# AntoineRichard/MoonSuperResolution

Hardware: AMD Instinct MI355X
Metric: 512x512 DEM tiles/s (whole job) (higher is better)
Workload: dtype f16 main term + fp8 / fp6 cross terms in the chip-filling convs, bf16x3 elsewhere (f32 in/out/accumulate; parity mode); 1 GPU; SPADE-512 GauGAN(512,8,256) batch=8 512x512 tiles per step (BASELINE configs[2]); image_size=512, batch_size=8, variant=gaugan, weights=random-init (Keras default distributions), seed 1234, parallelism=tile-sharded x1, streams_per_gpu=1

## Files before the change

### moonsuperresolution_amd/csrc/conv_sw.hip

```cpp
#include "conv_common.h"

namespace msr {

struct SwGeom {
    int tiles_x, tiles_y, tiles_n, tiles_mn;
    int walk_pb, walk_nb;
};

static constexpr int SW_HW = 18, SW_HP = 18 * 18, SW_BKP = 40, SW_HPB = SW_HP * SW_BKP;
#ifdef MSR_SW_STAMPS
static constexpr size_t SW_LDS = (size_t)3 * SW_HPB * sizeof(float) + 8192;
#else
static constexpr size_t SW_LDS = (size_t)3 * SW_HPB * sizeof(float);
#endif

template <int EPI, int OS>
__device__ __forceinline__ void sw_epilogue_body(const ConvParams& p, const SwGeom& g, f32x4 (&acc)[16][2], int wq, int lane,
                                                 int n0, int tx0, int ty0, int b0) {
    const int px = lane & 15, cg = lane >> 4;
    const int x = tx0 + px;
    const int cb0 = n0 + (wq >> 1) * 64 + (wq & 1) * 16 + 4 * cg;
    float* const obase = p.out + (size_t)p.out_off + (size_t)b0 * p.out_pb + x * p.out_px;
    if constexpr (EPI == EPI_SPADE) {
        const int ch = ((n0 + (wq >> 1) * 64) >> 1) + (wq & 1) * 16 + 4 * cg;
        const float4 gq4 = *reinterpret_cast<const float4*>(p.bias + cb0);
        const float4 bq4 = *reinterpret_cast<const float4*>(p.bias + cb0 + 32);
        const float4 mq4 = *reinterpret_cast<const float4*>(p.mean + ch);
        const float4 sq4 = *reinterpret_cast<const float4*>(p.stdv + ch);
        const float gq[4] = {gq4.x, gq4.y, gq4.z, gq4.w}, bq[4] = {bq4.x, bq4.y, bq4.z, bq4.w};
        const float mq[4] = {mq4.x, mq4.y, mq4.z, mq4.w};
        float sq[4] = {sq4.x, sq4.y, sq4.z, sq4.w};
        constexpr bool split = OS != OUT_F32;
        if constexpr (split) {
#pragma unroll
            for (int k = 0; k < 4; ++k) sq[k] = 1.f / sq[k];
        }
        const float* const abase = p.aux + (size_t)b0 * p.aux_pb + (x >> p.aux_shift) * p.aux_px + ch;
#pragma unroll
        for (int i0 = 0; i0 < 16; i0 += 8) {
            float4 xin[8];
#pragma unroll
            for (int ii = 0; ii < 8; ++ii)
                xin[ii] = *reinterpret_cast<const float4*>(abase + ((ty0 + i0 + ii) >> p.aux_shift) * p.aux_py);
#pragma unroll
            for (int ii = 0; ii < 8; ++ii) {
                const int i = i0 + ii;
                float* orow = obase + (ty0 + i) * p.out_py;
                const float xq[4] = {xin[ii].x, xin[ii].y, xin[ii].z, xin[ii].w};
                float v[4];
#pragma unroll
                for (int k = 0; k < 4; ++k) {
                    const float normalized = split ? (xq[k] - mq[k]) * sq[k] : (xq[k] - mq[k]) / sq[k];
                    const float t = (acc[i][0][k] + gq[k]) * normalized + (acc[i][1][k] + bq[k]);
                    v[k] = t >= 0.f ? t : t * p.slope;
                }
                if constexpr (OS == OUT_F16C) msr_store_f16c4_dev(orow, ch, v[0], v[1], v[2], v[3]);
                else if constexpr (OS == OUT_BF16X3) msr_store_split4_dev(orow, ch, v[0], v[1], v[2], v[3]);
                else *reinterpret_cast<float4*>(orow + ch) = make_float4(v[0], v[1], v[2], v[3]);
            }
        }
    } else {
#pragma unroll
        for (int j = 0; j < 2; ++j) {
            const int col = cb0 + 32 * j;
            const float4 b4 = *reinterpret_cast<const float4*>(p.bias + col);
            const float bq[4] = {b4.x, b4.y, b4.z, b4.w};
#pragma unroll
            for (int q4 = 0; q4 < 4; ++q4) {
                float4 res[4];
                if constexpr (EPI == EPI_RES) {
                    const float* abase = p.aux + (size_t)b0 * p.aux_pb + (x >> p.aux_shift) * p.aux_px + col;
#pragma unroll
                    for (int ii = 0; ii < 4; ++ii)
                        res[ii] = *reinterpret_cast<const float4*>(abase + ((ty0 + q4 * 4 + ii) >> p.aux_shift) * p.aux_py);
                }
                float s1[4] = {0.f, 0.f, 0.f, 0.f}, s2[4] = {0.f, 0.f, 0.f, 0.f}, pv[4];
#pragma unroll
                for (int ii = 0; ii < 4; ++ii) {
                    const int i = q4 * 4 + ii;
                    float d[4];
#pragma unroll
                    for (int k = 0; k < 4; ++k) d[k] = acc[i][j][k];
                    if constexpr (EPI == EPI_RES) { d[0] += res[ii].x; d[1] += res[ii].y; d[2] += res[ii].z; d[3] += res[ii].w; }
                    *reinterpret_cast<float4*>(obase + (ty0 + i) * p.out_py + col) =
                        make_float4(d[0] + bq[0], d[1] + bq[1], d[2] + bq[2], d[3] + bq[3]);
#pragma unroll
                    for (int k = 0; k < 4; ++k) {
                        if (ii == 0) pv[k] = d[k];
                        const float e = d[k] - pv[k];
                        s1[k] += e; s2[k] += e * e;
                    }
                }
                if (p.stat_partial) {
                    float mean[4], m2[4];
#pragma unroll
                    for (int k = 0; k < 4; ++k) {
                        const float mu = row16_sum(4.f * pv[k] + s1[k]) * (1.f / 64.f);
                        const float dl = (pv[k] - mu) + s1[k] * 0.25f;
                        const float t = row16_sum(s2[k] - s1[k] * s1[k] * 0.25f + 4.f * dl * dl);
                        mean[k] = bq[k] + mu;
                        m2[k] = t > 0.f ? t : 0.f;
                    }
                    if (px == 0) {
                        const int st = (b0 * (g.tiles_y * 2) + ((ty0 + q4 * 4) >> 3)) * g.tiles_x + (tx0 >> 4);
                        float* o = p.stat_partial + (size_t)(st * 2 + (q4 & 1)) * 3 * p.N + col;
                        *reinterpret_cast<float4*>(o) = make_float4(64.f, 64.f, 64.f, 64.f);
                        *reinterpret_cast<float4*>(o + p.N) = make_float4(mean[0], mean[1], mean[2], mean[3]);
                        *reinterpret_cast<float4*>(o + 2 * p.N) = make_float4(m2[0], m2[1], m2[2], m2[3]);
                    }
                }
            }
        }
    }
}

template <int EPI>
__device__ __forceinline__ void sw_epilogue(const ConvParams& p, const SwGeom& g, f32x4 (&acc)[16][2], int wq, int lane,
                                            int n0, int tx0, int ty0, int b0) {
    if constexpr (EPI == EPI_SPADE) {
        if (p.out_split == OUT_F16C) sw_epilogue_body<EPI, OUT_F16C>(p, g, acc, wq, lane, n0, tx0, ty0, b0);
        else if (p.out_split == OUT_BF16X3) sw_epilogue_body<EPI, OUT_BF16X3>(p, g, acc, wq, lane, n0, tx0, ty0, b0);
        else sw_epilogue_body<EPI, OUT_F32>(p, g, acc, wq, lane, n0, tx0, ty0, b0);
    } else {
        sw_epilogue_body<EPI, OUT_F32>(p, g, acc, wq, lane, n0, tx0, ty0, b0);
    }
}

#ifdef SW_NOBAR
#define SW_BARRIER() {}
#else
#define SW_BARRIER()                                           \
    {                                                          \
        __builtin_amdgcn_fence(__ATOMIC_RELEASE, "workgroup"); \
        __builtin_amdgcn_s_barrier();                          \
        __builtin_amdgcn_fence(__ATOMIC_ACQUIRE, "workgroup"); \
    }
#endif
#ifndef SW_UNROLL2
#define SW_UNROLL2 1
#endif
#ifndef SW_PD
#define SW_PD 6
#endif
#ifndef SW_PDC
#define SW_PDC 3
#endif

template <int EPI, bool F6 = false, bool NOX = false>
__global__ void __launch_bounds__(256) __attribute__((amdgpu_waves_per_eu(1, 1)))
conv_igemm_f16c_sw(const ConvParams p, const SwGeom g) {
    MSR_SATURATING_CONVERSIONS();
    constexpr int HW = SW_HW, HP = SW_HP, BKP = SW_BKP, HPB = SW_HPB;
    constexpr int NTHR = 256, BKC = 32;
    constexpr int H_ITEMS = (HP * 8 + NTHR - 1) / NTHR;
    static_assert(H_ITEMS == 11, "halo staging is written for 11 items per thread");
    constexpr int PD = SW_PD;
    constexpr int PDC = SW_PDC;
    constexpr int HD = 3;

    extern __shared__ __attribute__((aligned(16))) float smem[];

    const int tid = threadIdx.x;
    const int lane = tid & 63;
    const int wq = __builtin_amdgcn_readfirstlane(tid >> 6);
    const int px = lane & 15, cg = lane >> 4;

    int slots, cnt, base;
    xcd_tile_range(g.tiles_mn, slots, cnt, base);
    int tile = blockIdx.x >> 3;
    if (tile >= cnt) return;

    int n0, tx0, ty0, b0;
    unsigned h_tile, w_tile;
#define SW_DECODE(T_, N0_, TX_, TY_, B_, HT_, WT_)                                               \
    {                                                                                            \
        const int t_ = (T_);                                                                     \
        int tn_, tmi_;                                                                           \
        MSR_WALK(g, t_, tn_, tmi_)                                                               \
        TX_ = (tmi_ % g.tiles_x) << 4;                                                           \
        tmi_ /= g.tiles_x;                                                                       \
        TY_ = (tmi_ % g.tiles_y) << 4;                                                           \
        B_ = tmi_ / g.tiles_y;                                                                   \
        N0_ = tn_ * 128;                                                                         \
        HT_ = (unsigned)((B_) * p.in_pb + (TY_) * p.in_py + (TX_) * p.Cin) * 4u;                 \
        WT_ = (unsigned)((N0_) * p.Cin) * 4u;                                                    \
    }
    SW_DECODE(base + tile, n0, tx0, ty0, b0, h_tile, w_tile)

    const int hp0 = tid >> 3, hseg = tid & 7;
    const int h_l0 = hp0 * BKP + hseg * 4;
    const bool h_live = !NOX || hseg < 4;
#define SW_HPIX(q) ((q) < 10 ? hp0 + 32 * (q) : min(hp0 + 32 * (q), HP - 1))
#define SW_HGOFF(q) ((((SW_HPIX(q) * 3641) >> 16) * p.in_py + (SW_HPIX(q) - ((SW_HPIX(q) * 3641) >> 16) * HW) * p.Cin + hseg * 4) * 4)
#define SW_HLOFF(q) ((q) < 10 ? h_l0 + 32 * (q) * BKP : SW_HPIX(q) * BKP + hseg * 4)
    int b_voff[2], b_xoff[2];
#pragma unroll
    for (int j = 0; j < 2; ++j) {
        const int row_ = (((wq >> 1) * 64 + (wq & 1) * 16 + 32 * j + px) * p.Cin) * 4;
        b_voff[j] = row_ + 16 * cg;
        b_xoff[j] = F6 ? row_ + 64 + 32 * (cg & 1) : row_ + 16 * cg + 64;
    }
    const int a_lane = px * BKP + 4 * cg;
    const int x_lane = px * BKP + 16 + 8 * (cg & 1);

    const unsigned w_tap_bytes = (unsigned)((size_t)p.N * p.Cin * sizeof(float));
    const __amdgpu_buffer_rsrc_t rs_in = __builtin_amdgcn_make_buffer_rsrc(
        const_cast<float*>(p.in), 0, (int)((size_t)p.B * p.in_pb * sizeof(float)), 0x00020000);
    const __amdgpu_buffer_rsrc_t rs_wt = __builtin_amdgcn_make_buffer_rsrc(
        const_cast<float*>(p.wt), 0, (int)(9u * w_tap_bytes), 0x00020000);
#define SW_BUFLD(rs, voff, soff) __builtin_amdgcn_raw_buffer_load_b128(rs, voff, (int)(soff), 0)

    const int asc = (cg & 1) ? 0x74747474 : 0x7F7F7F7F;
    int wsc[2];
    f32x4 acc[16][2];
    i32x4 bE[2], bO[2], xE[2], xO[2], nbE[2], nbO[2], nxE[2], nxO[2];
    i32x4 fa[16], fb[16], ce[16], co[16];
    i32x4 rh[HD][2];

    const int ppi = p.Cin / (2 * BKC);
    int rb = 0;

#define SW_WSOFF(T) ((T) < 18 ? w_cur + (unsigned)((T) / 9) * (BKC * 4) + (unsigned)((T) % 9) * w_tap_bytes \
                              : w_after + (unsigned)((T) - 18) * w_tap_bytes)
#define SW_LOAD_B(dstE, dstO, dxE, dxO, T, j)                                                    \
    {                                                                                            \
        dstE[j] = SW_BUFLD(rs_wt, b_voff[j], SW_WSOFF(T));                                       \
        dstO[j] = SW_BUFLD(rs_wt, b_voff[j], SW_WSOFF((T) + 1));                                 \
        if constexpr (NOX) {                                                                     \
        } else if constexpr (F6) {                                                                      \
             \
            const unsigned lo_ = min(SW_WSOFF(T), SW_WSOFF((T) + 1));                            \
            const int dv_ = (int)((cg < 2 ? SW_WSOFF(T) : SW_WSOFF((T) + 1)) - lo_);             \
            dxE[j] = SW_BUFLD(rs_wt, b_xoff[j] + dv_, lo_);                                      \
            dxO[j] = SW_BUFLD(rs_wt, b_xoff[j] + dv_ + 16, lo_);                                 \
        } else {                                                                                 \
            dxE[j] = SW_BUFLD(rs_wt, b_xoff[j], SW_WSOFF(T));                                    \
            dxO[j] = SW_BUFLD(rs_wt, b_xoff[j], SW_WSOFF((T) + 1));                              \
        }                                                                                        \
    }
#define SW_APTR(T) ((T) < 9 ? A0 : (T) < 18 ? A1 : A2)
#define SW_AOFF(T, i) ((((i) + (((T) % 9) / 3)) * HW + (((T) % 9) % 3)) * BKP)
#define SW_RD_F(dst, T, i) dst = *reinterpret_cast<const i32x4*>(SW_APTR(T) + SW_AOFF(T, i))
#define SW_RD_X(dst, T, i) dst = *reinterpret_cast<const i32x4*>(SW_APTR(T) + SW_AOFF(T, i) + 16)
#define SW_XP(TE) ((cg < 2 ? SW_APTR(TE) + SW_AOFF(TE, 0) : SW_APTR((TE) + 1) + SW_AOFF((TE) + 1, 0)) - a_lane + x_lane)
#define SW_RD_X6(dlo, dhi, XP, i)                                                                \
    {                                                                                            \
        dlo = *reinterpret_cast<const i32x4*>((XP) + (i) * HW * BKP);                            \
        dhi = *reinterpret_cast<const i32x4*>((XP) + (i) * HW * BKP + 4);                        \
    }
#define SW_F16(v) __builtin_bit_cast(f16x8, v)
#define SW_CAT8(lo, hi) __builtin_shufflevector(lo, hi, 0, 1, 2, 3, 4, 5, 6, 7)
#define SW_HALO(T)                                                                               \
    {                                                                                            \
        constexpr int t_ = (T) % 9;                                                              \
        float* const w_ = (T) < 9 ? W1 : W2;                                                     \
        const unsigned hs_ = (T) < 9 ? h_cur + BKC * 4 : h_after;                                \
        if constexpr (t_ >= HD && t_ <= 5 + HD) {                                                \
            constexpr int q_ = 2 * (t_ - HD);                                                    \
            if (h_live) {                                                                        \
            *reinterpret_cast<i32x4*>(w_ + SW_HLOFF(q_)) = rh[(t_ - HD) % HD][0];                \
            if constexpr (q_ + 1 < H_ITEMS) *reinterpret_cast<i32x4*>(w_ + SW_HLOFF((q_ + 1) % H_ITEMS)) = rh[(t_ - HD) % HD][1]; \
            }                                                                                    \
        }                                                                                        \
        if constexpr (t_ <= 5) {                                                                 \
            if (h_live) {                                                                        \
            rh[t_ % HD][0] = SW_BUFLD(rs_in, SW_HGOFF(2 * t_), hs_);                             \
            if constexpr (2 * t_ + 1 < H_ITEMS) rh[t_ % HD][1] = SW_BUFLD(rs_in, SW_HGOFF((2 * t_ + 1) % H_ITEMS), hs_); \
            }                                                                                    \
        }                                                                                        \
    }
#ifdef MSR_SW_STAMPS
    unsigned* const dbg = reinterpret_cast<unsigned*>(smem + 3 * HPB) + wq * 64;
    int dbg_n = 0;
    bool dbg_on = false;
    if (lane == 0) dbg[63] = 0;
#define SW_STAMP(LVL)                                                                            \
    if (MSR_SW_STAMPS >= (LVL) && dbg_on && lane == 0 && dbg_n < 64) dbg[dbg_n++] = (unsigned)__builtin_amdgcn_s_memtime();
#else
#define SW_STAMP(LVL)
#endif
#define SW_PHASE_E(U)                                                                            \
    {                                                                                            \
        constexpr int T = 2 * (U);                                                               \
        SW_STAMP(1)                                                                              \
        SW_HALO(T)                                                                               \
        _Pragma("unroll") for (int i = 0; i < 16; ++i) {                                         \
            if (T + 1 == 9 && i == 16 - PD) SW_BARRIER()                                         \
            if (i + PD < 16) SW_RD_F(fa[(i + PD) & 15], T, (i + PD) & 15);                       \
            else SW_RD_F(fb[(i + PD) & 15], T + 1, (i + PD) & 15);                               \
            if (i == 0) SW_LOAD_B(nbE, nbO, nxE, nxO, T + 2, 0)                                  \
            if (i == 8) SW_LOAD_B(nbE, nbO, nxE, nxO, T + 2, 1)                                  \
            acc[i][0] = __builtin_amdgcn_mfma_f32_16x16x32_f16(SW_F16(bE[0]), SW_F16(fa[i]), acc[i][0], 0, 0, 0); \
            acc[i][1] = __builtin_amdgcn_mfma_f32_16x16x32_f16(SW_F16(bE[1]), SW_F16(fa[i]), acc[i][1], 0, 0, 0); \
            __builtin_amdgcn_sched_barrier(0);                                                   \
        }                                                                                        \
    }
#define SW_PHASE_O(U)                                                                            \
    {                                                                                            \
        constexpr int T = 2 * (U) + 1;                                                           \
        SW_STAMP(2)                                                                              \
        SW_HALO(T)                                                                               \
        const float* const xp_ = SW_XP(T - 1);                                                   \
        _Pragma("unroll") for (int i = 0; i < 16; ++i) {                                         \
            if (i + PD < 16) SW_RD_F(fb[(i + PD) & 15], T, (i + PD) & 15);                       \
            if constexpr (NOX) {     \
                if (T + 1 == 18 && i == 16 - PD) SW_BARRIER()                                    \
                if (i >= 16 - PD) SW_RD_F(fa[(i + PD) & 15], T + 1, (i + PD) & 15);              \
            } else if (i >= 16 - PDC) {                                                          \
                if constexpr (F6) {                                                              \
                    SW_RD_X6(ce[(i + PDC) & 15], co[(i + PDC) & 15], xp_, (i + PDC) & 15)        \
                } else {                                                                         \
                    SW_RD_X(ce[(i + PDC) & 15], T - 1, (i + PDC) & 15);                          \
                    SW_RD_X(co[(i + PDC) & 15], T, (i + PDC) & 15);                              \
                }                                                                                \
            }                                                                                    \
            acc[i][0] = __builtin_amdgcn_mfma_f32_16x16x32_f16(SW_F16(bO[0]), SW_F16(fb[i]), acc[i][0], 0, 0, 0); \
            acc[i][1] = __builtin_amdgcn_mfma_f32_16x16x32_f16(SW_F16(bO[1]), SW_F16(fb[i]), acc[i][1], 0, 0, 0); \
            __builtin_amdgcn_sched_barrier(0);                                                   \
        }                                                                                        \
    }
#define SW_PHASE_C(U)                                                                            \
    {                                                                                            \
        constexpr int T = 2 * (U);                                                               \
        SW_STAMP(2)                                                                              \
        const i32x8 wq0_ = SW_CAT8(xE[0], xO[0]), wq1_ = SW_CAT8(xE[1], xO[1]);                  \
        const float* const xp_ = SW_XP(T);                                                       \
        if constexpr (!NOX) {                                                                    \
        _Pragma("unroll") for (int i = 0; i < 16; ++i) {                                         \
            if (T + 2 == 18 && i == 16 - PD) SW_BARRIER()                                        \
            if (i + PDC < 16) {                                                                  \
                if constexpr (F6) {                                                              \
                    SW_RD_X6(ce[(i + PDC) & 15], co[(i + PDC) & 15], xp_, (i + PDC) & 15)        \
                } else {                                                                         \
                    SW_RD_X(ce[(i + PDC) & 15], T, (i + PDC) & 15);                              \
                    SW_RD_X(co[(i + PDC) & 15], T + 1, (i + PDC) & 15);                          \
                }                                                                                \
            }                                                                                    \
            if (i >= 16 - PD) SW_RD_F(fa[(i + PD) & 15], T + 2, (i + PD) & 15);                  \
            const i32x8 aq_ = SW_CAT8(ce[i], co[i]);                                             \
            if constexpr (F6) {      \
                acc[i][0] = __builtin_amdgcn_mfma_scale_f32_16x16x128_f8f6f4(wq0_, aq_, acc[i][0], 2, 2, 0, wq0_[6], 0, aq_[6]); \
                acc[i][1] = __builtin_amdgcn_mfma_scale_f32_16x16x128_f8f6f4(wq1_, aq_, acc[i][1], 2, 2, 0, wq1_[6], 0, aq_[6]); \
            } else {                                                                             \
                acc[i][0] = __builtin_amdgcn_mfma_scale_f32_16x16x128_f8f6f4(wq0_, aq_, acc[i][0], 0, 0, 0, wsc[0], 0, asc); \
                acc[i][1] = __builtin_amdgcn_mfma_scale_f32_16x16x128_f8f6f4(wq1_, aq_, acc[i][1], 0, 0, 0, wsc[1], 0, asc); \
            }                                                                                    \
            __builtin_amdgcn_sched_barrier(0);                                                   \
        }                                                                                        \
        }                                                                                        \
        _Pragma("unroll") for (int j = 0; j < 2; ++j) { bE[j] = nbE[j]; bO[j] = nbO[j]; xE[j] = nxE[j]; xO[j] = nxO[j]; } \
    }
#define SW_PAIR(U) SW_PHASE_E(U) SW_PHASE_O(U) SW_PHASE_C(U)
#define SW_BODY() SW_PAIR(0) SW_PAIR(1) SW_PAIR(2) SW_PAIR(3) SW_PAIR(4) SW_PAIR(5) SW_PAIR(6) SW_PAIR(7) SW_PAIR(8)
#define SW_SETUP(PR, LAST)                                                                       \
    const unsigned w_cur = w_tile + (unsigned)(PR) * (2 * BKC * 4);                              \
    const unsigned h_cur = h_tile + (unsigned)(PR) * (2 * BKC * 4);                              \
    const unsigned w_after = (LAST) ? w_next : w_cur + 2 * BKC * 4;                              \
    const unsigned h_after = (LAST) ? h_next : h_cur + 2 * BKC * 4;                              \
    const int r1 = rb == 2 ? 0 : rb + 1, r2 = r1 == 2 ? 0 : r1 + 1;                              \
    const float* const A0 = smem + rb * HPB + a_lane;                                            \
    const float* const A1 = smem + r1 * HPB + a_lane;                                            \
    const float* const A2 = smem + r2 * HPB + a_lane;                                            \
    float* const W1 = smem + r1 * HPB;                                                           \
    float* const W2 = smem + r2 * HPB;

    {
        i32x4 t[H_ITEMS];
#pragma unroll
        for (int q = 0; q < H_ITEMS; ++q) if (h_live) t[q] = SW_BUFLD(rs_in, SW_HGOFF(q), h_tile);
#pragma unroll
        for (int q = 0; q < H_ITEMS; ++q) if (h_live) *reinterpret_cast<i32x4*>(smem + SW_HLOFF(q)) = t[q];
    }
    {
        const unsigned w_cur = w_tile, w_after = w_tile;
        SW_LOAD_B(bE, bO, xE, xO, 0, 0)
        SW_LOAD_B(bE, bO, xE, xO, 0, 1)
    }
    SW_BARRIER()
    {
        const float* const A0 = smem + a_lane;
        const float* const A1 = A0;
        const float* const A2 = A0;
#pragma unroll
        for (int i = 0; i < PD; ++i) SW_RD_F(fa[i], 0, i);
    }

    for (;;) {
        const int tnext = tile + slots;
        const bool has_next = tnext < cnt;
        int n0n, tx0n, ty0n, b0n;
        unsigned h_next, w_next;
        SW_DECODE(base + (has_next ? tnext : tile), n0n, tx0n, ty0n, b0n, h_next, w_next)
#pragma unroll
        for (int i = 0; i < 16; ++i)
#pragma unroll
            for (int j = 0; j < 2; ++j)
#pragma unroll
                for (int r = 0; r < 4; ++r) acc[i][j][r] = 0.f;
#pragma unroll
        for (int j = 0; j < 2; ++j) {
            const int w_ = F6 ? 0 : p.wexp[n0 + (wq >> 1) * 64 + (wq & 1) * 16 + 32 * j + px];
            wsc[j] = (((cg & 1) ? (w_ >> 8) : w_) & 0xFF) * 0x01010101;
        }
#if SW_UNROLL2
        for (int pr = 0; pr < ppi; pr += 2) {
            { SW_SETUP(pr, false) SW_BODY() rb = r2; }
            { SW_SETUP(pr + 1, pr + 2 == ppi) SW_BODY() rb = r2; }
        }
#else
        for (int pr = 0; pr < ppi; ++pr) {
            SW_SETUP(pr, pr == ppi - 1)
#ifdef MSR_SW_STAMPS
            dbg_on = blockIdx.x == 8 && pr == (ppi > 2 ? 2 : 1) && dbg_n == 0;
#endif
            SW_BODY()
            SW_STAMP(1)
#ifdef MSR_SW_STAMPS
            dbg_on = false;
#endif
            rb = r2;
        }
#endif
#ifdef MSR_SW_STAMPS
        const unsigned te0_ = (unsigned)__builtin_amdgcn_s_memtime();
#endif
#ifdef SW_NOEPI
        if (p.B < 0)
#endif
        sw_epilogue<EPI>(p, g, acc, wq, lane, n0, tx0, ty0, b0);
#ifdef MSR_SW_STAMPS
        if (blockIdx.x == 8 && lane == 0 && dbg_n > 0 && dbg_n < 63 && dbg[63] == 0) dbg[63] = (unsigned)__builtin_amdgcn_s_memtime() - te0_;
#endif
        if (!has_next) break;
        tile = tnext;
        n0 = n0n; tx0 = tx0n; ty0 = ty0n; b0 = b0n;
        h_tile = h_next;
        w_tile = w_next;
    }
#ifdef MSR_SW_STAMPS
    if (blockIdx.x == 8 && lane == 0) {
        for (int k = 0; k + 1 < dbg_n; ++k) printf("wave %d stamp %2d: %5u cycles\n", wq, k, dbg[k + 1] - dbg[k]);
        printf("wave %d body total %u, epilogue (issue) %u\n", wq, dbg[dbg_n - 1] - dbg[0], dbg[63]);
    }
#endif
#undef SW_STAMP
#undef SW_DECODE
#undef SW_HPIX
#undef SW_HGOFF
#undef SW_HLOFF
#undef SW_BUFLD
#undef SW_WSOFF
#undef SW_LOAD_B
#undef SW_APTR
#undef SW_AOFF
#undef SW_RD_F
#undef SW_RD_X
#undef SW_XP
#undef SW_RD_X6
#undef SW_F16
#undef SW_CAT8
#undef SW_HALO
#undef SW_PHASE_E
#undef SW_PHASE_O
#undef SW_PHASE_C
#undef SW_PAIR
#undef SW_BODY
#undef SW_SETUP
}

hipError_t conv_sw_init() {
    hipError_t e;
#define SW_SET(EPI)                                                                                          \
    if ((e = hipFuncSetAttribute(reinterpret_cast<const void*>(&conv_igemm_f16c_sw<EPI>),                    \
                                 hipFuncAttributeMaxDynamicSharedMemorySize, (int)SW_LDS)) != hipSuccess)    \
        return e;
    SW_SET(EPI_BIAS) SW_SET(EPI_RES) SW_SET(EPI_SPADE)
#undef SW_SET
    if ((e = hipFuncSetAttribute(reinterpret_cast<const void*>(&conv_igemm_f16c_sw<EPI_BIAS, true>),
                                 hipFuncAttributeMaxDynamicSharedMemorySize, (int)SW_LDS)) != hipSuccess) return e;
    if ((e = hipFuncSetAttribute(reinterpret_cast<const void*>(&conv_igemm_f16c_sw<EPI_RES, true>),
                                 hipFuncAttributeMaxDynamicSharedMemorySize, (int)SW_LDS)) != hipSuccess) return e;
    if ((e = hipFuncSetAttribute(reinterpret_cast<const void*>(&conv_igemm_f16c_sw<EPI_BIAS, false, true>),
                                 hipFuncAttributeMaxDynamicSharedMemorySize, (int)SW_LDS)) != hipSuccess) return e;
    if ((e = hipFuncSetAttribute(reinterpret_cast<const void*>(&conv_igemm_f16c_sw<EPI_RES, false, true>),
                                 hipFuncAttributeMaxDynamicSharedMemorySize, (int)SW_LDS)) != hipSuccess) return e;
    return hipSuccess;
}

hipError_t launch_conv_f16c_sw(const ConvParams& p, int epi, hipStream_t s) {
    auto pow2 = [](int v) { return v > 0 && (v & (v - 1)) == 0; };
    if (epi == EPI_SPADE && p.out_split != OUT_F32 && p.out_split != OUT_BF16X3 && p.out_split != OUT_F16C) return hipErrorInvalidValue;
    const bool f6 = p.prec == PREC_F16C6;
    if ((p.prec != PREC_F16C && !f6) || (!f6 && !p.wexp) || p.ksplit > 1 || p.stride != 1 || p.KH != 3 || p.KW != 3) return hipErrorInvalidValue;
    if (f6 && epi == EPI_SPADE) return hipErrorInvalidValue;
    if (!pow2(p.Hout) || !pow2(p.Wout) || p.Hout < 16 || p.Wout < 16 || p.N % 128 || p.Cin % (SW_UNROLL2 ? 128 : 64)) return hipErrorInvalidValue;
    if ((size_t)p.B * p.in_pb * sizeof(float) >= ((size_t)1 << 31)) return hipErrorInvalidValue;
    SwGeom g;
    g.tiles_x = p.Wout / 16;
    g.tiles_y = p.Hout / 16;
    g.tiles_n = p.N / 128;
    g.tiles_mn = g.tiles_x * g.tiles_y * p.B * g.tiles_n;
    conv_walk_pick(g.tiles_x * g.tiles_y * p.B, g.tiles_n, &g.walk_pb, &g.walk_nb);
    const int grid = persistent_grid(g.tiles_mn);
    if (!grid) return hipErrorInvalidValue;
    if (f6) {
        if (epi == EPI_BIAS) conv_igemm_f16c_sw<EPI_BIAS, true><<<grid, 256, SW_LDS, s>>>(p, g);
        else conv_igemm_f16c_sw<EPI_RES, true><<<grid, 256, SW_LDS, s>>>(p, g);
        return hipGetLastError();
    }
    if (p.no_cross) {
        if (epi == EPI_BIAS) conv_igemm_f16c_sw<EPI_BIAS, false, true><<<grid, 256, SW_LDS, s>>>(p, g);
        else if (epi == EPI_RES) conv_igemm_f16c_sw<EPI_RES, false, true><<<grid, 256, SW_LDS, s>>>(p, g);
        else return hipErrorInvalidValue;
        return hipGetLastError();
    }
    switch (epi) {
        case EPI_BIAS: conv_igemm_f16c_sw<EPI_BIAS><<<grid, 256, SW_LDS, s>>>(p, g); break;
        case EPI_RES: conv_igemm_f16c_sw<EPI_RES><<<grid, 256, SW_LDS, s>>>(p, g); break;
        case EPI_SPADE: conv_igemm_f16c_sw<EPI_SPADE><<<grid, 256, SW_LDS, s>>>(p, g); break;
        default: return hipErrorInvalidValue;
    }
    return hipGetLastError();
}

}
```

Measured before the change: 912.0 tiles/s.

## Batch residual prefetch and defer moment reductions in conv epilogue

The residual/plain conv epilogue is restructured into one loop over 8 row-groups. For residual layers it issues all 16 residual float4 loads up front, reads accumulators explicitly from AGPRs, and defers each group's cross-lane moment reduction by one group so that shuffles overlap the next group's add and store. The aim is to hide residual-load latency and row16_sum shuffle latency. In exchange it holds 32 float4 residual registers live, which raises VGPR pressure and may hurt occupancy. It also adds optional timing stamps and a profiling script.

Result: no change. 911.9 tiles/s (-0.0%).

```diff
diff --git a/moonsuperresolution_amd/csrc/conv_sw.hip b/moonsuperresolution_amd/csrc/conv_sw.hip
--- a/moonsuperresolution_amd/csrc/conv_sw.hip
+++ b/moonsuperresolution_amd/csrc/conv_sw.hip
@@ -14,9 +14,64 @@
 static constexpr size_t SW_LDS = (size_t)3 * SW_HPB * sizeof(float);
 #endif
 
+#ifndef SW_RES_ROWS
+#define SW_RES_ROWS 16
+#endif
+#ifndef SW_EPI_DEFER
+#define SW_EPI_DEFER 1
+#endif
+#ifdef MSR_SW_STAMPS
+#define SW_EST_PARAM , unsigned (&et)[4]
+#define SW_EST_ARG , et
+#define SW_ESTAMP_BEGIN() unsigned et_last_ = (unsigned)__builtin_amdgcn_s_memtime();
+#define SW_ESTAMP_WAIT() __builtin_amdgcn_s_waitcnt(0x0F70);
+#define SW_ESTAMP(K)                                                   \
+    {                                                                  \
+        __builtin_amdgcn_sched_barrier(0);                             \
+        const unsigned t_ = (unsigned)__builtin_amdgcn_s_memtime();    \
+        et[K] += t_ - et_last_;                                        \
+        et_last_ = t_;                                                 \
+        __builtin_amdgcn_sched_barrier(0);                             \
+    }
+#else
+#define SW_EST_PARAM
+#define SW_EST_ARG
+#define SW_ESTAMP_BEGIN()
+#define SW_ESTAMP_WAIT()
+#define SW_ESTAMP(K)
+#endif
+
+__device__ __forceinline__ float sw_acc_read(float a) {
+    float v;
+    asm("v_accvgpr_read_b32 %0, %1" : "=v"(v) : "a"(a));
+    return v;
+}
+
+__device__ __forceinline__ void sw_moment_slab(const ConvParams& p, const SwGeom& g, const float (&s1)[4], const float (&s2)[4],
+                                               const float (&pv)[4], const float (&bq)[4], int px, int cb0, int tx0, int ty0,
+                                               int b0, int gi) {
+    const int q4 = gi & 3, col = cb0 + 32 * (gi >> 2);
+    float mean[4], m2[4];
+#pragma unroll
+    for (int k = 0; k < 4; ++k) {
+        const float mu = row16_sum(4.f * pv[k] + s1[k]) * (1.f / 64.f);
+        const float dl = (pv[k] - mu) + s1[k] * 0.25f;
+        const float t = row16_sum(s2[k] - s1[k] * s1[k] * 0.25f + 4.f * dl * dl);
+        mean[k] = bq[k] + mu;
+        m2[k] = t > 0.f ? t : 0.f;
+    }
+    if (px == 0) {
+        const int st = (b0 * (g.tiles_y * 2) + ((ty0 + q4 * 4) >> 3)) * g.tiles_x + (tx0 >> 4);
+        float* o = p.stat_partial + (size_t)(st * 2 + (q4 & 1)) * 3 * p.N + col;
+        *reinterpret_cast<float4*>(o) = make_float4(64.f, 64.f, 64.f, 64.f);
+        *reinterpret_cast<float4*>(o + p.N) = make_float4(mean[0], mean[1], mean[2], mean[3]);
+        *reinterpret_cast<float4*>(o + 2 * p.N) = make_float4(m2[0], m2[1], m2[2], m2[3]);
+    }
+}
+
 template <int EPI, int OS>
 __device__ __forceinline__ void sw_epilogue_body(const ConvParams& p, const SwGeom& g, f32x4 (&acc)[16][2], int wq, int lane,
-                                                 int n0, int tx0, int ty0, int b0) {
+                                                 int n0, int tx0, int ty0, int b0 SW_EST_PARAM) {
     const int px = lane & 15, cg = lane >> 4;
     const int x = tx0 + px;
     const int cb0 = n0 + (wq >> 1) * 64 + (wq & 1) * 16 + 4 * cg;
@@ -60,69 +115,84 @@
             }
         }
     } else {
-#pragma unroll
-        for (int j = 0; j < 2; ++j) {
+        constexpr bool RES = EPI == EPI_RES;
+        constexpr int RB = SW_RES_ROWS;
+        constexpr bool DEFER = RES && SW_EPI_DEFER;
+        static_assert(RB == 4 || RB == 8 || RB == 16 || RB == 32, "SW_RES_ROWS: whole 4-row groups of the tile's 2 x 16 rows");
+        float4 res[RES ? 32 : 1];
+        const char* abase = nullptr;
+        unsigned a_lane = 0;
+        if constexpr (RES) {
+            abase = reinterpret_cast<const char*>(p.aux + (size_t)b0 * p.aux_pb);
+            a_lane = (unsigned)((x >> p.aux_shift) * p.aux_px + cb0) * 4u;
+        }
+        float bq[4], s1p[4], s2p[4], pvp[4], bqp[4];
+        SW_ESTAMP_BEGIN()
+#pragma unroll
+        for (int gi = 0; gi < 8; ++gi) {
+            const int j = gi >> 2, q4 = gi & 3;
             const int col = cb0 + 32 * j;
-            const float4 b4 = *reinterpret_cast<const float4*>(p.bias + col);
-            const float bq[4] = {b4.x, b4.y, b4.z, b4.w};
-#pragma unroll
-            for (int q4 = 0; q4 < 4; ++q4) {
-                float4 res[4];
-                if constexpr (EPI == EPI_RES) {
-                    const float* abase = p.aux + (size_t)b0 * p.aux_pb + (x >> p.aux_shift) * p.aux_px + col;
-#pragma unroll
-                    for (int ii = 0; ii < 4; ++ii)
-                        res[ii] = *reinterpret_cast<const float4*>(abase + ((ty0 + q4 * 4 + ii) >> p.aux_shift) * p.aux_py);
-                }
-                float s1[4] = {0.f, 0.f, 0.f, 0.f}, s2[4] = {0.f, 0.f, 0.f, 0.f}, pv[4];
-#pragma unroll
-                for (int ii = 0; ii < 4; ++ii) {
-                    const int i = q4 * 4 + ii;
-                    float d[4];
-#pragma unroll
-                    for (int k = 0; k < 4; ++k) d[k] = acc[i][j][k];
-                    if constexpr (EPI == EPI_RES) { d[0] += res[ii].x; d[1] += res[ii].y; d[2] += res[ii].z; d[3] += res[ii].w; }
-                    *reinterpret_cast<float4*>(obase + (ty0 + i) * p.out_py + col) =
-                        make_float4(d[0] + bq[0], d[1] + bq[1], d[2] + bq[2], d[3] + bq[3]);
-#pragma unroll
-                    for (int k = 0; k < 4; ++k) {
-                        if (ii == 0) pv[k] = d[k];
-                        const float e = d[k] - pv[k];
-                        s1[k] += e; s2[k] += e * e;
-                    }
-                }
-                if (p.stat_partial) {
-                    float mean[4], m2[4];
-#pragma unroll
-                    for (int k = 0; k < 4; ++k) {
-                        const float mu = row16_sum(4.f * pv[k] + s1[k]) * (1.f / 64.f);
-                        const float dl = (pv[k] - mu) + s1[k] * 0.25f;
-                        const float t = row16_sum(s2[k] - s1[k] * s1[k] * 0.25f + 4.f * dl * dl);
-                        mean[k] = bq[k] + mu;
-                        m2[k] = t > 0.f ? t : 0.f;
-                    }
-                    if (px == 0) {
-                        const int st = (b0 * (g.tiles_y * 2) + ((ty0 + q4 * 4) >> 3)) * g.tiles_x + (tx0 >> 4);
-                        float* o = p.stat_partial + (size_t)(st * 2 + (q4 & 1)) * 3 * p.N + col;
-                        *reinterpret_cast<float4*>(o) = make_float4(64.f, 64.f, 64.f, 64.f);
-                        *reinterpret_cast<float4*>(o + p.N) = make_float4(mean[0], mean[1], mean[2], mean[3]);
-                        *reinterpret_cast<float4*>(o + 2 * p.N) = make_float4(m2[0], m2[1], m2[2], m2[3]);
-                    }
+            if (q4 == 0) {
+                const float4 b4 = *reinterpret_cast<const float4*>(p.bias + col);
+                bq[0] = b4.x; bq[1] = b4.y; bq[2] = b4.z; bq[3] = b4.w;
+                if (RES && gi > 0) __builtin_amdgcn_sched_barrier(0);
+            }
+            if constexpr (RES) {
+                if ((4 * gi) % RB == 0) {
+#pragma unroll
+                    for (int m = 4 * gi; m < 4 * gi + RB; ++m)
+                        res[m] = *reinterpret_cast<const float4*>(
+                            abase + ((size_t)(((ty0 + (m & 15)) >> p.aux_shift) * p.aux_py) * 4 + 128 * (m >> 4)) + a_lane);
+                    __builtin_amdgcn_sched_barrier(0);
+                    SW_ESTAMP_WAIT()
+                    SW_ESTAMP(0)
                 }
             }
-        }
+            float s1[4] = {0.f, 0.f, 0.f, 0.f}, s2[4] = {0.f, 0.f, 0.f, 0.f}, pv[4];
+#pragma unroll
+            for (int ii = 0; ii < 4; ++ii) {
+                const int i = q4 * 4 + ii;
+                float d[4];
+#pragma unroll
+                for (int k = 0; k < 4; ++k) d[k] = RES ? sw_acc_read(acc[i][j][k]) : acc[i][j][k];
+                if constexpr (RES) {
+                    const float4 r4 = res[4 * gi + ii];
+                    d[0] += r4.x; d[1] += r4.y; d[2] += r4.z; d[3] += r4.w;
+                }
+                *reinterpret_cast<float4*>(obase + (ty0 + i) * p.out_py + col) =
+                    make_float4(d[0] + bq[0], d[1] + bq[1], d[2] + bq[2], d[3] + bq[3]);
+#pragma unroll
+                for (int k = 0; k < 4; ++k) {
+                    if (ii == 0) pv[k] = d[k];
+                    const float e = d[k] - pv[k];
+                    s1[k] += e; s2[k] += e * e;
+                }
+            }
+            SW_ESTAMP(1)
+            if constexpr (DEFER) {
+                if (gi > 0 && p.stat_partial) sw_moment_slab(p, g, s1p, s2p, pvp, bqp, px, cb0, tx0, ty0, b0, gi - 1);
+#pragma unroll
+                for (int k = 0; k < 4; ++k) { s1p[k] = s1[k]; s2p[k] = s2[k]; pvp[k] = pv[k]; bqp[k] = bq[k]; }
+                if (gi == 7 && p.stat_partial) sw_moment_slab(p, g, s1p, s2p, pvp, bqp, px, cb0, tx0, ty0, b0, gi);
+            } else {
+                if (p.stat_partial) sw_moment_slab(p, g, s1, s2, pv, bq, px, cb0, tx0, ty0, b0, gi);
+            }
+            SW_ESTAMP(2)
+        }
+        SW_ESTAMP_WAIT()
+        SW_ESTAMP(3)
     }
 }
 
 template <int EPI>
 __device__ __forceinline__ void sw_epilogue(const ConvParams& p, const SwGeom& g, f32x4 (&acc)[16][2], int wq, int lane,
-                                            int n0, int tx0, int ty0, int b0) {
+                                            int n0, int tx0, int ty0, int b0 SW_EST_PARAM) {
     if constexpr (EPI == EPI_SPADE) {
-        if (p.out_split == OUT_F16C) sw_epilogue_body<EPI, OUT_F16C>(p, g, acc, wq, lane, n0, tx0, ty0, b0);
-        else if (p.out_split == OUT_BF16X3) sw_epilogue_body<EPI, OUT_BF16X3>(p, g, acc, wq, lane, n0, tx0, ty0, b0);
-        else sw_epilogue_body<EPI, OUT_F32>(p, g, acc, wq, lane, n0, tx0, ty0, b0);
+        if (p.out_split == OUT_F16C) sw_epilogue_body<EPI, OUT_F16C>(p, g, acc, wq, lane, n0, tx0, ty0, b0 SW_EST_ARG);
+        else if (p.out_split == OUT_BF16X3) sw_epilogue_body<EPI, OUT_BF16X3>(p, g, acc, wq, lane, n0, tx0, ty0, b0 SW_EST_ARG);
+        else sw_epilogue_body<EPI, OUT_F32>(p, g, acc, wq, lane, n0, tx0, ty0, b0 SW_EST_ARG);
     } else {
-        sw_epilogue_body<EPI, OUT_F32>(p, g, acc, wq, lane, n0, tx0, ty0, b0);
+        sw_epilogue_body<EPI, OUT_F32>(p, g, acc, wq, lane, n0, tx0, ty0, b0 SW_EST_ARG);
     }
 }
 
@@ -422,14 +492,18 @@
         }
 #endif
 #ifdef MSR_SW_STAMPS
+        unsigned et[4] = {0u, 0u, 0u, 0u};
         const unsigned te0_ = (unsigned)__builtin_amdgcn_s_memtime();
 #endif
 #ifdef SW_NOEPI
         if (p.B < 0)
 #endif
-        sw_epilogue<EPI>(p, g, acc, wq, lane, n0, tx0, ty0, b0);
-#ifdef MSR_SW_STAMPS
-        if (blockIdx.x == 8 && lane == 0 && dbg_n > 0 && dbg_n < 63 && dbg[63] == 0) dbg[63] = (unsigned)__builtin_amdgcn_s_memtime() - te0_;
+        sw_epilogue<EPI>(p, g, acc, wq, lane, n0, tx0, ty0, b0 SW_EST_ARG);
+#ifdef MSR_SW_STAMPS
+        if (blockIdx.x == 8 && lane == 0 && dbg_n > 0 && dbg_n < 56 && dbg[63] == 0) {
+            dbg[63] = (unsigned)__builtin_amdgcn_s_memtime() - te0_;
+            for (int k = 0; k < 4; ++k) dbg[56 + k] = et[k];
+        }
 #endif
         if (!has_next) break;
         tile = tnext;
@@ -441,6 +515,9 @@
     if (blockIdx.x == 8 && lane == 0) {
         for (int k = 0; k + 1 < dbg_n; ++k) printf("wave %d stamp %2d: %5u cycles\n", wq, k, dbg[k + 1] - dbg[k]);
         printf("wave %d body total %u, epilogue (issue) %u\n", wq, dbg[dbg_n - 1] - dbg[0], dbg[63]);
+        if (EPI != EPI_SPADE)
+            printf("wave %d epilogue epi=%d r=%d cin=%d N=%d rows=%d defer=%d: residual wait %u, add+store issue %u, moments %u, store drain %u\n",
+                   wq, EPI, p.Hout, p.Cin, p.N, SW_RES_ROWS, SW_EPI_DEFER, dbg[56], dbg[57], dbg[58], dbg[59]);
     }
 #endif
 #undef SW_STAMP
diff --git a/profiles/layer_spread.py b/profiles/layer_spread.py
--- /dev/null
+++ b/profiles/layer_spread.py
@@ -0,0 +1,23 @@
+import csv
+import sys
+
+rows = [r for r in csv.DictReader(open(sys.argv[1])) if "msr::" in r["Kernel_Name"]]
+rows.sort(key=lambda r: int(r["Start_Timestamp"]))
+calls, K = int(sys.argv[2]), int(sys.argv[3])
+pats = sys.argv[4:] or ["conv_igemm_f16c_sw", "head_kernel"]
+n = len(rows) // calls
+assert n * calls == len(rows), (len(rows), calls)
+print(f"{n} launches per call, statistics over the last {K} of {calls} calls (us)")
+print(f"{'slot':>4s} {'mean':>8s} {'min':>8s} {'max':>8s} {'spread':>7s}  kernel")
+total = [0.0] * K
+for slot in range(n):
+    name = rows[(calls - 1) * n + slot]["Kernel_Name"].split("(")[0].replace("void msr::", "").replace("msr::", "")
+    d = []
+    for c in range(calls - K, calls):
+        r = rows[c * n + slot]
+        d.append((int(r["End_Timestamp"]) - int(r["Start_Timestamp"])) / 1e3)
+    for i, v in enumerate(d):
+        total[i] += v
+    if any(p in name for p in pats):
+        print(f"{slot:4d} {sum(d) / K:8.1f} {min(d):8.1f} {max(d):8.1f} {max(d) - min(d):7.1f}  {name}")
+print(f"sum of all kernel durations per call: mean {sum(total) / K:.1f} min {min(total):.1f} max {max(total):.1f}")
```
